# emtiyaz/vmp-for-svae

Hardware: AMD Instinct MI355X
Metric: vmp_step_datapoints_per_sec (higher is better)
Workload: dtype f32

## Files before the change

vmp-for-svae_amd/csrc/vmp_mix.hip:

```cpp
#include "vmp_common.h"
#include "vmp_linalg.h"
#include <stdlib.h>
#include <type_traits>

using namespace vmp;

namespace {

constexpr int TR = 64;
constexpr int LS = 68;
constexpr int MAX_NW = 8;
constexpr int MAX_NW1 = 8;
constexpr int max_nw(int KT) { return KT == 1 ? MAX_NW1 : MAX_NW; }
constexpr int MAX_BLOCKS = 1024;

struct PassArgs {
    const float* x;
    const float* r_in;
    const float* u_in;
    const uint8_t* mask;
    const float* pivot;
    const float* pack;
    float* r_out;
    float* u_out;
    float* logr_out;
    double* partials;
    long long N;
    long long rpw;
    long long rpw_b;
    int K;
    int vec_ok;
    int par_reduce;
#ifdef VMP_DEBUG_TS
    long long* dbg_t;
#endif
};
#ifdef VMP_DEBUG_TS
#define PASS_TS(i) do { if (a.dbg_t && (blockIdx.x == 0 || blockIdx.x == 100) && (threadIdx.x & 63) == 0) { a.dbg_t[(blockIdx.x ? 64 : 0) + (threadIdx.x >> 6) * 8 + (i)] = clock64(); \
    if ((i) == 0 && threadIdx.x == 0) a.dbg_t[(blockIdx.x ? 64 : 0) + 7] = wall_clock64();           \
    if ((i) == 5 && threadIdx.x == 64) a.dbg_t[(blockIdx.x ? 64 : 0) + 8 + 7] = wall_clock64(); } } while (0)
#else
#define PASS_TS(i) do { } while (0)
#endif

#define VMP_DPP2(OP, CTRL)                                                   \
    "v_" OP "_f32_dpp %0, %0, %0 " CTRL " row_mask:0xf bank_mask:0xf\n\t"  \
    "v_" OP "_f32_dpp %1, %1, %1 " CTRL " row_mask:0xf bank_mask:0xf\n\t"  \
    "s_nop 0\n\t"
#define VMP_DPP2_FIRST(OP, CTRL)                                             \
    "v_" OP "_f32_dpp %0, %2, %2 " CTRL " row_mask:0xf bank_mask:0xf\n\t"  \
    "v_" OP "_f32_dpp %1, %3, %3 " CTRL " row_mask:0xf bank_mask:0xf\n\t"  \
    "s_nop 0\n\t"
__device__ __forceinline__ v2f row16_max2(v2f v) {
    float a, b;
    asm("s_nop 1\n\t" VMP_DPP2_FIRST("max", "row_ror:8") VMP_DPP2("max", "row_ror:4") VMP_DPP2("max", "row_ror:2")
// ... 456 lines not shown
#pragma unroll
                for (int kt = 0; kt < KT; ++kt) {
#pragma unroll
                    for (int c = 0; c < 4; ++c) {
                        if constexpr (SMM) dn[kt][c] += (double)nacc[kt][c] + (double)nacs[kt][c];
#pragma unroll
                        for (int ft = 0; ft < FT; ++ft) dacc[kt][ft][c] += (double)acc[kt][ft][c] + (double)acs[kt][ft][c];
                    }
                    nacc[kt] = f32x4{0.f, 0.f, 0.f, 0.f};
                    nacs[kt] = f32x4{0.f, 0.f, 0.f, 0.f};
#pragma unroll
                    for (int ft = 0; ft < FT; ++ft) { acc[kt][ft] = f32x4{0.f, 0.f, 0.f, 0.f}; acs[kt][ft] = f32x4{0.f, 0.f, 0.f, 0.f}; }
                }
            }
        }
        __builtin_amdgcn_wave_barrier();
    }

    PASS_TS(2);
    if constexpr (STATS) pass_epilogue<D, KT, FLAV>(a, smem, dacc, dn, lane, wave, nw);
}


constexpr int AIS = 36;

struct FinArgs {
    const double* partials;
    const double* stats_in;
    int nblk, K, flavour, src, do_post;
    const float *alpha0, *beta0, *m0, *C0, *v0, *kappa;
    const float* pivot;
    float *alpha, *beta, *m, *C, *v, *xbar, *S, *pi, *pack;
    double* pack64;
    double* stats_out;
    double* peer[VMP_EXCH_MAX_RANKS];
    int nranks, rank;
    unsigned long long iter;
    int* status;
#ifdef VMP_DEBUG_TS
    long long* dbg_t;
#endif
};

#ifdef VMP_DEBUG_TS
#define FIN_TS(i) do { if (a.dbg_t && blockIdx.x == 0 && tid == 0) { a.dbg_t[i] = clock64(); if ((i) == 0) a.dbg_t[6] = wall_clock64(); if ((i) == 5) a.dbg_t[7] = wall_clock64(); } } while (0)
#else
#define FIN_TS(i) do { } while (0)
#endif

template <int D>
__device__ void finalize_block(const FinArgs& a, const int k, const int tid, const int nthreads);

template <int D> constexpr int xdl_wave_floats() { return Geo<D>::XROWS * LS + TR * AIS; }

template <int D, int FLAV, bool STATS, int MT = 3>
__device__ __forceinline__ void pass_xdl_body(const PassArgs& a) {
    using G = Geo<D>;
    constexpr int FT = G::FT, KT = 1;
    constexpr bool SMM = (FLAV == VMP_SMM);
    constexpr int DP = (D + 1) / 2;
    extern __shared__ __attribute__((aligned(16))) float smem[];
    const int lane = threadIdx.x & 63, wave = threadIdx.x >> 6, nw = blockDim.x >> 6;
    const int K = a.K;
    PASS_TS(0);
    float* xl = smem + wave * xdl_wave_floats<D>();
    unsigned* ai = reinterpret_cast<unsigned*>(xl + G::XROWS * LS);
    constexpr int ONE = D, ZERO = D + 1;
    const int ppos = (lane & ~15) + 4 * (lane & 3) + ((lane >> 2) & 3);
    xl[ONE * LS + lane] = 1.0f;
    xl[ZERO * LS + lane] = 0.0f;
    {
        u32x4 ones = u32x4{0x3F803F80u, 0x00003F80u, 0u, 0u}, zeros = u32x4{0u, 0u, 0u, 0u};
        *reinterpret_cast<u32x4*>(ai + lane * AIS + 12) = ones;
        *reinterpret_cast<u32x4*>(ai + lane * AIS + 16) = zeros;
    }

    const bool vec = a.vec_ok != 0;
    long long lo, hi;
    if (a.rpw_b == a.rpw) {
        lo = ((long long)blockIdx.x * nw + wave) * a.rpw;
        hi = lo + a.rpw;
    } else {
        const int hw = nw >> 1;
        const long long base = (long long)blockIdx.x * hw * (a.rpw + a.rpw_b);
        lo = wave < hw ? base + wave * a.rpw : base + hw * a.rpw + (wave - hw) * a.rpw_b;
        hi = lo + (wave < hw ? a.rpw : a.rpw_b);
    }
    if (hi > a.N) hi = a.N;
    float xr[D];
    {
        const long long n = lo + lane;
#pragma unroll
        for (int j = 0; j < D; ++j) xr[j] = 0.f;
        if (n < hi) load_row<D>(a.x + n * D, xr, vec);
    }
    const int i16 = lane & 15, kk = lane >> 4;
    float pv[D];
    {
        const float* __restrict__ pp = a.pivot ? a.pivot : a.x;
        const bool hasp = a.pivot != nullptr;
#pragma unroll
        for (int j = 0; j < D; ++j) { const float v = pp[j]; pv[j] = hasp ? v : 0.f; }
    }

    constexpr int NS = D < 4 ? D : 4;
    constexpr int NB = D > 4 ? D - 4 : 0;
    u32x4 Bsm[NS], B1[NB > 0 ? NB : 1], B2[NB > 0 ? NB : 1];
    v2f pch;
    float pua, pub;
    {
        const bool on = i16 < K;
        const float* __restrict__ p = a.pack + (on ? i16 : 0) * G::PACK;
        float raw[G::PACK];
        if (G::PACK % 4 == 0 && (reinterpret_cast<uintptr_t>(a.pack) & 15) == 0) {
#pragma unroll
            for (int j = 0; j < G::PACK / 4; ++j) {
                const float4 q = reinterpret_cast<const float4*>(p)[j];
                raw[4 * j] = q.x; raw[4 * j + 1] = q.y; raw[4 * j + 2] = q.z; raw[4 * j + 3] = q.w;
            }
        } else {
#pragma unroll
            for (int j = 0; j < G::PACK; ++j) raw[j] = p[j];
        }
        pch.x = on ? raw[D + G::TRI] : -INFINITY;
        pch.y = on ? raw[D + G::TRI + 1] : 0.f;
        pua = on ? raw[D + G::TRI + 2] : 0.f;
        pub = on ? raw[D + G::TRI + 3] : 1.f;
#pragma unroll
        for (int i = 0; i < D; ++i) {
            double bi = 0.0;
#pragma unroll
            for (int j = 0; j <= i; ++j) bi -= (double)raw[D + i * (i + 1) / 2 + j] * ((double)raw[j] - (double)pv[j]);
            unsigned tb[3];
            split_bf16<3>(v2f{(float)bi, 0.f}, tb);
            const unsigned bias0 = (tb[0] & 0xffffu) | (tb[1] << 16), bias1 = tb[2] & 0xffffu;
            unsigned th[4] = {0u, 0u, 0u, 0u}, tm[4] = {0u, 0u, 0u, 0u}, tl[4] = {0u, 0u, 0u, 0u};
#pragma unroll
            for (int q = 0; q < DP; ++q) {
                const int j0 = 2 * q, j1 = 2 * q + 1;
                const float wa = j0 <= i ? raw[D + i * (i + 1) / 2 + j0] : 0.f;
                const float wb = (j1 <= i && j1 < D) ? raw[D + i * (i + 1) / 2 + (j1 <= i ? j1 : 0)] : 0.f;
                unsigned t3[3];
                split_bf16<3>(v2f{wa, wb}, t3);
                th[q] = t3[0]; tm[q] = t3[1]; tl[q] = t3[2];
            }
            if (i < NS) {
                const u32x4 w = kk == 0 ? u32x4{th[0], th[1], tm[0], tm[1]}
                              : kk == 1 ? u32x4{th[0], th[1], tl[0], tl[1]}
                              : kk == 2 ? u32x4{th[0], th[1], tm[0], tm[1]}
                                        : u32x4{bias0, bias1, 0u, 0u};
                Bsm[i] = on ? w : u32x4{0u, 0u, 0u, 0u};
            } else {
                const int ib = i - 4;
                const u32x4 w1 = kk == 0 ? u32x4{th[0], th[1], th[2], th[3]} : kk == 1 ? u32x4{bias0, bias1, 0u, 0u}
                               : kk == 2 ? u32x4{tm[0], tm[1], tm[2], tm[3]} : u32x4{th[0], th[1], th[2], th[3]};
                const u32x4 w2 = kk == 0 ? u32x4{tl[0], tl[1], tl[2], tl[3]} : kk == 1 ? u32x4{th[0], th[1], th[2], th[3]}
                               : kk == 2 ? u32x4{tm[0], tm[1], tm[2], tm[3]} : u32x4{0u, 0u, 0u, 0u};
                B1[ib < 0 ? 0 : ib] = on ? w1 : u32x4{0u, 0u, 0u, 0u};
                B2[ib < 0 ? 0 : ib] = on ? w2 : u32x4{0u, 0u, 0u, 0u};
            }
        }
    }
    const int rho = 4 * (i16 & 3) + (i16 >> 2);
    const int offA1 = rho * AIS + (kk == 1 ? 12 : (kk == 3 ? 4 : 0));
    const int offA2 = rho * AIS + (kk == 0 ? 0 : (kk == 1 ? 8 : (kk == 2 ? 4 : 16)));
    const int offA3 = rho * AIS + (kk == 3 ? 12 : 20 + 4 * kk);

    int offA[FT], offB[FT];
#pragma unroll
    for (int ft = 0; ft < FT; ++ft) {
        const int f = ft * 16 + i16;
        int ra = ZERO, rb = ZERO;
        if (f == 0) { ra = ONE; rb = ONE; }
        else if (f <= D) { ra = f - 1; rb = ONE; }
        else if (f < G::F) {
            int p = f - D - 1, d = 0;
            while (p >= D - d) { p -= D - d; ++d; }
            ra = d; rb = d + p;
        }
        offA[ft] = ra * LS + 4 * kk;
        offB[ft] = rb * LS + 4 * kk;
    }

    f32x4 acc[KT][FT], acs[KT][FT];
    double dacc[KT][FT][4];
    double dn[KT][4];
    float nsum = 0.f;
    double dnl = 0.0;
#pragma unroll
    for (int c = 0; c < 4; ++c) dn[0][c] = 0.0;
#pragma unroll
    for (int ft = 0; ft < FT; ++ft) {
        acc[0][ft] = f32x4{0.f, 0.f, 0.f, 0.f};
        acs[0][ft] = f32x4{0.f, 0.f, 0.f, 0.f};
#pragma unroll
// ... 266 lines not shown
        double acc = (i == lane) ? 1.0 : 0.0;
#pragma unroll
        for (int p = 0; p < i; ++p) acc -= readlane_d(row[p], i) * X[p];
        X[i] = acc * rd[i];
    }
}

template <int D>
__device__ void estep_constants(int k, int flavour, double alpha_k, double alpha_sum, double beta_k, double v_k,
                                double logdetP, double kap, double& c, double& h, double& ua, double& ub, double& elp) {
    const double LOG2 = 0.69314718055994530942, PI = 3.14159265358979323846;
    elp = digamma_d(alpha_k) - digamma_d(alpha_sum);
    double sdg = 0.0;
    if (flavour == VMP_GMM) {
        for (int i = 0; i < D; ++i) sdg += digamma_d(0.5 * (v_k + 1.0 + i));
        const double ld = (logdetP > log(1e-20)) ? logdetP : 0.0;
        const double eld = sdg + D * LOG2 + ld;
        c = elp + 0.5 * eld - 0.5 * (D / beta_k);
        h = 0.5; ua = 1.0; ub = 1.0;
    } else {
        for (int i = 0; i < D; ++i) sdg += digamma_d(0.5 * (v_k + i));
        const double eld = sdg + D * LOG2 + logdetP;
        h = 0.5 * (D + kap);
        c = lgamma(0.5 * (D + kap)) - lgamma(0.5 * kap) - 0.5 * D * log(kap * PI) + elp + 0.5 * eld
            - h * (D / beta_k) + log(kap);
        ua = D + kap;
        ub = D / beta_k + kap;
    }
}

constexpr int FIN_THREADS = 1024;
constexpr int FIN_MAX_GROUPS = FIN_THREADS / 64;

__device__ __forceinline__ void st_pack(const FinArgs& a, int idx, double v) {
    a.pack[idx] = (float)v;
    if (a.pack64) a.pack64[idx] = v;
}

template <int D>
__device__ void finalize_block(const FinArgs& a, const int k, const int tid, const int nthreads) {
    using G = Geo<D>;
    __shared__ double part[FIN_MAX_GROUPS][64];
    __shared__ double st[G::SW];
    __shared__ double ntot;
    __shared__ double Ck[D * D], mk[D], sp[D + 4], scal[8];
    __shared__ double alpha0s[VMP_MAX_K];
    const int K = a.K;
    const int FIN_GROUPS = nthreads >> 6;
    const bool post = a.do_post != 0;
    const bool smm = a.flavour == VMP_SMM;
    const double beta0 = post ? (double)a.beta0[k] : 0.0, v0 = post ? (double)a.v0[k] : 0.0;
    const double alpha0 = post ? (double)a.alpha0[k] : 0.0;
    const double kap = (post && smm) ? (double)a.kappa[k] : 0.0;
    bool shifted = (a.src == 0) && (a.pivot != nullptr);
    double m0d = 0.0, m0e = 0.0, C0de = 0.0, cd = 0.0, ce = 0.0;
    if (tid < D * D) {
        const int d = tid / D, e = tid % D;
        if (post) { m0d = a.m0[k * D + d]; m0e = a.m0[k * D + e]; C0de = a.C0[(k * D + d) * D + e]; }
        if (shifted) { cd = a.pivot[d]; ce = a.pivot[e]; }
    }
    if (post && tid < K) alpha0s[tid] = a.alpha0[tid];

    FIN_TS(0);
    if (a.src == 0) {
        constexpr int PX = G::PF + 1;
        const int f = tid & 63, g = tid >> 6;
        const double* __restrict__ mine = a.partials + (long long)k * MAX_BLOCKS * PX;
        for (int lg = g; lg < FIN_MAX_GROUPS; lg += FIN_GROUPS) {
            double s = 0.0;
            for (int b0 = lg; b0 < a.nblk; b0 += FIN_MAX_GROUPS * 16) {
                double v1[16];
                const int fc = f < PX ? f : PX - 1;
#pragma unroll
                for (int i = 0; i < 16; ++i) {
                    const int b = b0 + i * FIN_MAX_GROUPS;
                    const int bc = b < a.nblk ? b : a.nblk - 1;
                    v1[i] = mine[(long long)bc * PX + fc];
                }
#pragma unroll
// ... 122 lines not shown
    const double v_k = smm ? (v0 + Nk) : (v0 + Nk + 1.0);
    FIN_TS(2);
    if (tid < D * D) {
        const int d = tid / D, e = tid % D;
        const double xd = empty ? sx[d] : sx[d] / den, xe = empty ? sx[e] : sx[e] / den;
        const double cen = sxx[d * D + e] - xd * sx[e] - sx[d] * xe + Wk * xd * xe;
        const double Sde = empty ? cen : cen / den;
        const double xrd = empty ? sx[d] + Wk * cd : xd + cd, xre = empty ? sx[e] + Wk * ce : xe + ce;
        const double q0d = xrd - m0d, q0e = xre - m0e;
        const double Cde = C0de + Wk * Sde + (beta0 * Wk / beta_k) * q0d * q0e;
        Ck[d * D + e] = Cde;
        if (a.S) a.S[(k * D + d) * D + e] = (float)Sde;
        if (a.C) a.C[(k * D + d) * D + e] = (float)Cde;
        if (e == 0) {
            const double md = (beta0 * m0d + Wk * xrd) / beta_k;
            mk[d] = md;
            if (a.m) a.m[k * D + d] = (float)md;
            if (a.xbar) a.xbar[k * D + d] = (float)xrd;
        }
    }
    if (tid == 0) {
        if (a.alpha) a.alpha[k] = (float)alpha_k;
        if (a.beta) a.beta[k] = (float)beta_k;
        if (a.v) a.v[k] = (float)v_k;
    }
    __syncthreads();
    FIN_TS(3);
    if (tid < 64) {
        double X[D], sumlog;
        bool ok;
        wave_chol_inverse<D>(Ck, tid, X, sumlog, ok);
        const double sv = ok ? sqrt(v_k) : nan("");
        if (a.pack && tid < D) {
            const int p = k * G::PACK + D;
#pragma unroll
            for (int i = 0; i < D; ++i)
                if (i >= tid) st_pack(a, p + i * (i + 1) / 2 + tid, X[i] * sv);
        }
        if (tid == 0) { scal[0] = -2.0 * sumlog; scal[1] = ok ? 1.0 : 0.0; }
    } else if (tid >= 64 && tid < 64 + D + 2) {
        const int i = tid - 64;
        double arg = 0.5 * (v_k + (smm ? 0.0 : 1.0) + i);
        if (i == D) arg = alpha_k;
        if (i == D + 1) {
            double asum = 0.0;
            for (int j = 0; j < K; ++j) asum += alpha0s[j];
            arg = asum + ntot;
        }
        sp[i] = digamma_d(arg);
    } else if (tid == 128 && smm) {
        sp[D + 2] = lgamma(0.5 * (D + kap)) - lgamma(0.5 * kap);
    }
    __syncthreads();
    FIN_TS(4);
    if (tid == 0) {
        const double LOG2 = 0.69314718055994530942, PI = 3.14159265358979323846;
        const double elp = sp[D] - sp[D + 1];
        double sdg = 0.0;
        for (int i = 0; i < D; ++i) sdg += sp[i];
        double c, h = 0.5, ua = 1.0, ub = 1.0;
        const double logdetP = scal[0];
        if (!smm) {
            const double ld = (logdetP > log(1e-20)) ? logdetP : 0.0;
            c = elp + 0.5 * (sdg + D * LOG2 + ld) - 0.5 * (D / beta_k);
        } else {
            h = 0.5 * (D + kap);
            c = sp[D + 2] - 0.5 * D * log(kap * PI) + elp + 0.5 * (sdg + D * LOG2 + logdetP) - h * (D / beta_k) + log(kap);
            ua = D + kap;
            ub = D / beta_k + kap;
        }
        if (scal[1] == 0.0) c = nan("");
        if (a.pi) a.pi[k] = (float)exp(elp);
        if (a.pack) {
            const int p = k * G::PACK + D + G::TRI;
            const double LOG2E = 1.4426950408889634074;
            st_pack(a, p, c * LOG2E); st_pack(a, p + 1, h * LOG2E); st_pack(a, p + 2, ua); st_pack(a, p + 3, ub);
        }
    }
    if (a.pack && tid < D) st_pack(a, k * G::PACK + tid, mk[tid]);
    FIN_TS(5);
}

template <int D>
__global__ __launch_bounds__(FIN_THREADS) void finalize_kernel(FinArgs a) {
    finalize_block<D>(a, blockIdx.x, threadIdx.x, FIN_THREADS);
}


struct PackArgs {
    int K, flavour;
    const float *alpha, *beta, *m, *P, *v, *kappa;
    float *pack, *pi;
};

template <int D>
__global__ void pack_kernel(PackArgs a) {
    const int k = blockIdx.x * blockDim.x + threadIdx.x;
    if (k >= a.K) return;
    double asum = 0.0;
    for (int j = 0; j < a.K; ++j) asum += a.alpha[j];
    const double v_k = a.v[k];
    double A[D * D], mk[D];
    for (int i = 0; i < D; ++i)
        for (int j = 0; j < D; ++j) {
            const int ri = D - 1 - i, rj = D - 1 - j;
            A[i * D + j] = 0.5 * ((double)a.P[(k * D + ri) * D + rj] + (double)a.P[(k * D + rj) * D + ri]);
        }
    double c = 0, h = 0.5, ua = 1, ub = 1, elp = 0;
    double W[D * D];
    if (chol_lower<D>(A)) {
        double ld = 0.0;
        for (int i = 0; i < D; ++i) ld += log(A[i * D + i]);
// ... 102 lines not shown
int launch_pass_dk(const PassArgs& a, const Plan& p, int flavour, bool estep, bool stats, bool mask, hipStream_t s) {
    dim3 grid(p.blocks), block(p.nw * WAVE);
#define VMP_LAUNCH(FL, E, S, M) \
    hipLaunchKernelGGL((pass_kernel<D, KT, FL, E, S, M>), grid, block, p.lds, s, a)
    if (flavour == VMP_GMM) {
        if (estep && stats) VMP_LAUNCH(VMP_GMM, true, true, false);
        else if (estep && mask) VMP_LAUNCH(VMP_GMM, true, false, true);
        else if (estep) VMP_LAUNCH(VMP_GMM, true, false, false);
        else VMP_LAUNCH(VMP_GMM, false, true, false);
    } else {
        if (estep && stats) VMP_LAUNCH(VMP_SMM, true, true, false);
        else if (estep) VMP_LAUNCH(VMP_SMM, true, false, false);
        else VMP_LAUNCH(VMP_SMM, false, true, false);
    }
#undef VMP_LAUNCH
    return check_launch("pass_kernel");
}

inline bool use_xdl(int K, bool estep, bool mask) { return estep && !mask && K <= 16; }

#ifndef VMP_MOM2_ROWS
#define VMP_MOM2_ROWS (1ll << 16)
#endif
template <int D>
int launch_pass_xdl(const PassArgs& a, const Plan& p, int flavour, bool stats, hipStream_t s) {
    dim3 grid(p.blocks), block(p.nw * WAVE);
#define VMP_LAUNCH_X(FL, S, M) do { \
        if (p.lds > 64 * 1024) { if (const int rc_ = set_dyn_lds(reinterpret_cast<const void*>(pass_xdl_kernel<D, FL, S, M>), p.lds, "pass_xdl_kernel")) return rc_; } \
        hipLaunchKernelGGL((pass_xdl_kernel<D, FL, S, M>), grid, block, p.lds, s, a); } while (0)
    const bool m2 = stats && a.N >= VMP_MOM2_ROWS;
    if (flavour == VMP_GMM) { if (m2) VMP_LAUNCH_X(VMP_GMM, true, 2); else if (stats) VMP_LAUNCH_X(VMP_GMM, true, 3); else VMP_LAUNCH_X(VMP_GMM, false, 3); }
    else { if (m2) VMP_LAUNCH_X(VMP_SMM, true, 2); else if (stats) VMP_LAUNCH_X(VMP_SMM, true, 3); else VMP_LAUNCH_X(VMP_SMM, false, 3); }
#undef VMP_LAUNCH_X
    return check_launch("pass_xdl_kernel");
}

template <int D>
int launch_pass_d(const PassArgs& a, const Plan& p, int flavour, bool estep, bool stats, bool mask, hipStream_t s) {
    if (use_xdl(a.K, estep, mask)) return launch_pass_xdl<D>(a, p, flavour, stats, s);
    const int KT = (a.K + 15) / 16;
    if (KT == 1) return launch_pass_dk<D, 1>(a, p, flavour, estep, stats, mask, s);
    if (KT == 2) return launch_pass_dk<D, 2>(a, p, flavour, estep, stats, mask, s);
    return launch_pass_dk<D, 4>(a, p, flavour, estep, stats, mask, s);
}

#define VMP_DISPATCH_D(D, CALL)            \
    switch (D) {                            \
        case 1: { constexpr int DD = 1; CALL; } break; \
        case 2: { constexpr int DD = 2; CALL; } break; \
        case 3: { constexpr int DD = 3; CALL; } break; \
        case 4: { constexpr int DD = 4; CALL; } break; \
        case 5: { constexpr int DD = 5; CALL; } break; \
        case 6: { constexpr int DD = 6; CALL; } break; \
        case 7: { constexpr int DD = 7; CALL; } break; \
        case 8: { constexpr int DD = 8; CALL; } break; \
        default: break;                     \
    }

int check_dims(int64_t N, int D, int K) {
    if (N <= 0) { set_error("N must be positive (got %lld)", (long long)N); return VMP_E_BADARG; }
    if (D < 1 || D > VMP_MAX_D) { set_error("D=%d outside compiled range 1..%d", D, VMP_MAX_D); return VMP_E_DIM; }
    if (K < 1 || K > VMP_MAX_K) { set_error("K=%d outside compiled range 1..%d", K, VMP_MAX_K); return VMP_E_DIM; }
    return 0;
}

bool aligned16(const void* p) { return (reinterpret_cast<uintptr_t>(p) & 15) == 0; }
// ... 128 lines not shown
            double s = 0.0;
            for (int n = 0; n < nr; ++n) {
                const double rr = (double)ws_[n * K + k];
                const double w = (smm && !isn[q]) ? rr * (double)us_[n * K + k] : rr;
                s = fma(w, (double)xs[n * XS + ia[q]] * (double)xs[n * XS + ib[q]], s);
            }
            acc[q] += s;
        }
    }
    __syncthreads();
    double* nk = reinterpret_cast<double*>(sm);
#pragma unroll
    for (int q = 0; q < ACC_ITEMS; ++q)
        if (ik[q] >= 0 && isn[q]) nk[ik[q]] = acc[q];
    __syncthreads();
    if (threadIdx.x == 0) {
        double t = 0.0;
        for (int k = 0; k < K; ++k) t += nk[k];
        nk[K] = t;
    }
    __syncthreads();
    constexpr int PX = G::PF + 1;
#pragma unroll
    for (int q = 0; q < ACC_ITEMS; ++q) {
        if (ik[q] < 0) continue;
        const int it = (int)threadIdx.x + q * ACC_THREADS, f = it - ik[q] * FP;
        double* row = a.partials + ((long long)ik[q] * MAX_BLOCKS + blockIdx.x) * PX;
        row[f] = acc[q];
        if (f == 0) row[G::PF] = nk[K];
    }
}

constexpr size_t WS_TPACK_WORDS = 16 * (VMP_MAX_D + VMP_MAX_D * (VMP_MAX_D + 1) / 2 + 4);
inline size_t ws_partial_bytes(int D, int K) { return (size_t)MAX_BLOCKS * K * (partial_words(D) + 1) * sizeof(double); }
inline unsigned long long* ws_seq(void* ws, int D, int K) { return reinterpret_cast<unsigned long long*>(static_cast<char*>(ws) + ws_partial_bytes(D, K)); }

}

extern "C" {

#ifdef VMP_DEBUG_TS
void vmp_debug_set_finalize_timestamps(long long* p) { g_dbg_t = p; }
void vmp_debug_set_pass_timestamps(long long* p) { g_dbg_pass = p; }
#endif

int vmp_mix_pack_words(int D) { return pack_words(D); }
int vmp_mix_stats_words(int D) { return stats_words(D); }

size_t vmp_mix_workspace_bytes(int64_t N, int D, int K) {
    (void)N;
    return ws_partial_bytes(D, K) + (WS_TPACK_WORDS + 2) * sizeof(unsigned long long);
}

int vmp_mix_pivot(const float* x, int64_t N, int D, float* pivot_out, void* stream) {
    int rc = check_dims(N, D, 1);
    if (rc) return rc;
    if (!x || !pivot_out) { set_error("vmp_mix_pivot: null pointer"); return VMP_E_BADARG; }
    PivotArgs a{x, N, D, pivot_out};
    hipLaunchKernelGGL(pivot_kernel, dim3(1), dim3(1024), 0, static_cast<hipStream_t>(stream), a);
    return check_launch("pivot_kernel");
}

int vmp_mix_stats(const float* x, const float* r, const float* u, const float* pivot, int64_t N, int D, int K,
                  double* stats, void* ws, size_t ws_bytes, void* stream) {
    int rc = check_dims(N, D, K);
    if (rc) return rc;
    if (!x || !r || !stats || !ws) { set_error("vmp_mix_stats: null pointer"); return VMP_E_BADARG; }
    if (ws_bytes < vmp_mix_workspace_bytes(N, D, K)) { set_error("vmp_mix_stats: workspace too small"); return VMP_E_WS; }
    hipStream_t s = static_cast<hipStream_t>(stream);
    if (N <= SMALL_STATS_MAX_N && !pivot) {
        SmallStatsArgs sa{x, r, u, stats, (int)N, D, K};
        hipLaunchKernelGGL(small_stats_kernel, dim3(K), dim3(SMALL_STATS_GROUPS * 80), 0, s, sa);
        return check_launch("small_stats_kernel");
    }
    const int flavour = u ? VMP_SMM : VMP_GMM;
    PassArgs a{};
    a.x = x; a.r_in = r; a.u_in = u; a.pivot = pivot; a.N = N; a.K = K; a.partials = static_cast<double*>(ws);
    a.vec_ok = aligned16(x) && aligned16(r) && (!u || aligned16(u));
    rc = run_pass(a, D, flavour, false, true, false, s);
    if (rc) return rc;
    FinArgs f{};
    f.partials = a.partials; f.nblk = make_plan(N, D, K, flavour, true).blocks; f.K = K; f.flavour = flavour;
    f.src = 0; f.do_post = 0; f.stats_out = stats; f.pivot = pivot;
    return run_finalize(f, D, s);
}

int vmp_mix_finalize(const double* stats, int D, int K, int flavour, const float* alpha0, const float* beta0,
                     const float* m0, const float* C0, const float* v0, const float* kappa, float* alpha, float* beta,
                     float* m, float* C, float* v, float* xbar, float* S, float* pi, float* pack, void* stream) {
    int rc = check_dims(1, D, K);
    if (rc) return rc;
    if (!stats || !alpha0 || !beta0 || !m0 || !C0 || !v0) { set_error("vmp_mix_finalize: null pointer"); return VMP_E_BADARG; }
    if (flavour == VMP_SMM && !kappa) { set_error("vmp_mix_finalize: SMM needs kappa"); return VMP_E_BADARG; }
    FinArgs f{};
    f.stats_in = stats; f.nblk = 0; f.K = K; f.flavour = flavour; f.src = 1; f.do_post = 1;
    f.alpha0 = alpha0; f.beta0 = beta0; f.m0 = m0; f.C0 = C0; f.v0 = v0; f.kappa = kappa;
    f.alpha = alpha; f.beta = beta; f.m = m; f.C = C; f.v = v; f.xbar = xbar; f.S = S; f.pi = pi; f.pack = pack;
    return run_finalize(f, D, static_cast<hipStream_t>(stream));
}

int vmp_mix_pack_from_params(int D, int K, int flavour, const float* alpha, const float* beta, const float* m,
                             const float* P, const float* v, const float* kappa, float* pack, float* pi, void* stream) {
    int rc = check_dims(1, D, K);
    if (rc) return rc;
    if (!alpha || !beta || !m || !P || !v || !pack) { set_error("vmp_mix_pack_from_params: null pointer"); return VMP_E_BADARG; }
    if (flavour == VMP_SMM && !kappa) { set_error("vmp_mix_pack_from_params: SMM needs kappa"); return VMP_E_BADARG; }
    PackArgs a{K, flavour, alpha, beta, m, P, v, kappa, pack, pi};
    hipStream_t s = static_cast<hipStream_t>(stream);
    rc = -1;
    VMP_DISPATCH_D(D, {
        hipLaunchKernelGGL((pack_kernel<DD>), dim3((K + 63) / 64), dim3(64), 0, s, a);
        rc = check_launch("pack_kernel");
    });
    return rc;
}

int vmp_mix_estep(const float* x, int64_t N, int D, int K, int flavour, const float* pack, const uint8_t* miss_mask,
                  float* r_out, float* u_out, float* logr_out, const float* pivot, double* stats_out, void* ws,
                  size_t ws_bytes, void* stream) {
    int rc = check_dims(N, D, K);
    if (rc) return rc;
    if (!x || !pack || !r_out) { set_error("vmp_mix_estep: null pointer"); return VMP_E_BADARG; }
    if (flavour == VMP_SMM && !u_out) { set_error("vmp_mix_estep: SMM needs u_out"); return VMP_E_BADARG; }
    if (flavour != VMP_GMM && flavour != VMP_SMM) { set_error("vmp_mix_estep: bad flavour %d", flavour); return VMP_E_BADARG; }
    if (miss_mask && (flavour != VMP_GMM || stats_out)) {
        set_error("vmp_mix_estep: miss_mask only with GMM flavour and without fused stats");
        return VMP_E_BADARG;
    }
    if (stats_out && (!ws || ws_bytes < vmp_mix_workspace_bytes(N, D, K))) {
        set_error("vmp_mix_estep: workspace too small for fused stats");
        return VMP_E_WS;
    }
    hipStream_t s = static_cast<hipStream_t>(stream);
    PassArgs a{};
    a.x = x; a.mask = miss_mask; a.pack = pack; a.r_out = r_out; a.u_out = u_out; a.logr_out = logr_out;
    a.pivot = pivot; a.N = N; a.K = K; a.partials = static_cast<double*>(ws);
    a.vec_ok = aligned16(x) && aligned16(r_out) && (!u_out || aligned16(u_out)) && (!logr_out || aligned16(logr_out));
    rc = run_pass(a, D, flavour, true, stats_out != nullptr, miss_mask != nullptr, s);
    if (rc || !stats_out) return rc;
    FinArgs f{};
    f.partials = a.partials; f.nblk = make_plan(N, D, K, flavour, true).blocks; f.K = K; f.flavour = flavour;
    f.src = 0; f.do_post = 0; f.stats_out = stats_out; f.pivot = pivot;
    return run_finalize(f, D, s);
}

int vmp_mix_estep_fused(const float* x, int64_t N, int D, int K, int flavour, const float* pack, float* r_out,
                        float* u_out, float* logr_out, const float* pivot, void* ws, size_t ws_bytes, void* stream) {
    int rc = check_dims(N, D, K);
    if (rc) return rc;
    if (!x || !pack || !r_out || !ws) { set_error("vmp_mix_estep_fused: null pointer"); return VMP_E_BADARG; }
    if (flavour != VMP_GMM && flavour != VMP_SMM) { set_error("vmp_mix_estep_fused: bad flavour %d", flavour); return VMP_E_BADARG; }
    if (flavour == VMP_SMM && !u_out) { set_error("vmp_mix_estep_fused: SMM needs u_out"); return VMP_E_BADARG; }
    if (ws_bytes < vmp_mix_workspace_bytes(N, D, K)) { set_error("vmp_mix_estep_fused: workspace too small"); return VMP_E_WS; }
    PassArgs a{};
    a.x = x; a.pack = pack; a.r_out = r_out; a.u_out = u_out; a.logr_out = logr_out; a.pivot = pivot;
    a.N = N; a.K = K; a.partials = static_cast<double*>(ws);
    a.vec_ok = aligned16(x) && aligned16(r_out) && (!u_out || aligned16(u_out)) && (!logr_out || aligned16(logr_out));
    return run_pass(a, D, flavour, true, true, false, static_cast<hipStream_t>(stream));
}

int vmp_mix_stats_ws(const float* x, const float* r, const float* u, const float* pivot, int64_t N, int D, int K,
                     void* ws, size_t ws_bytes, void* stream) {
    int rc = check_dims(N, D, K);
    if (rc) return rc;
    if (!x || !r || !ws) { set_error("vmp_mix_stats_ws: null pointer"); return VMP_E_BADARG; }
    if (ws_bytes < vmp_mix_workspace_bytes(N, D, K)) { set_error("vmp_mix_stats_ws: workspace too small"); return VMP_E_WS; }
    PassArgs a{};
    a.x = x; a.r_in = r; a.u_in = u; a.pivot = pivot; a.N = N; a.K = K; a.partials = static_cast<double*>(ws);
    a.vec_ok = aligned16(x) && aligned16(r) && (!u || aligned16(u));
    hipError_t e = hipMemsetAsync(ws_seq(ws, D, K), 0, (WS_TPACK_WORDS + 2) * sizeof(unsigned long long), static_cast<hipStream_t>(stream));
    if (e != hipSuccess) { set_error("vmp_mix_stats_ws: hipMemsetAsync: %s", hipGetErrorString(e)); return (int)e; }
    return run_pass(a, D, u ? VMP_SMM : VMP_GMM, false, true, false, static_cast<hipStream_t>(stream));
}

int vmp_mix_stats_ws_accurate(const float* x, const float* r, const float* u, const float* pivot, int64_t N, int D, int K,
                              void* ws, size_t ws_bytes, void* stream) {
    int rc = check_dims(N, D, K);
    if (rc) return rc;
    if (!x || !r || !ws) { set_error("vmp_mix_stats_ws_accurate: null pointer"); return VMP_E_BADARG; }
    if (ws_bytes < vmp_mix_workspace_bytes(N, D, K)) { set_error("vmp_mix_stats_ws_accurate: workspace too small"); return VMP_E_WS; }
    const int blocks = make_plan(N, D, K, u ? VMP_SMM : VMP_GMM, true).blocks;
    AccStatArgs a{x, r, u, pivot, static_cast<double*>(ws), N, (N + blocks - 1) / blocks, K};
    const size_t lds = (size_t)ACC_RS * (D + 1 + 2 * K) * sizeof(float);
    hipStream_t s = static_cast<hipStream_t>(stream);
    hipError_t e = hipMemsetAsync(ws_seq(ws, D, K), 0, (WS_TPACK_WORDS + 2) * sizeof(unsigned long long), s);
    if (e != hipSuccess) { set_error("vmp_mix_stats_ws_accurate: hipMemsetAsync: %s", hipGetErrorString(e)); return (int)e; }
    rc = -1;
    VMP_DISPATCH_D(D, {
        if (lds > 48 * 1024) { if ((rc = set_dyn_lds(reinterpret_cast<const void*>(stats_f64_kernel<DD>), lds, "stats_f64_kernel")) != 0) return rc; }
        hipLaunchKernelGGL((stats_f64_kernel<DD>), dim3(blocks), dim3(ACC_THREADS), lds, s, a);
        rc = check_launch("stats_f64_kernel");
    });
    return rc;
}

int vmp_mix_finalize_exchange(const void* ws, const float* pivot, int64_t N, int D, int K, int flavour, const float* alpha0,
                              const float* beta0, const float* m0, const float* C0, const float* v0, const float* kappa,
                              float* alpha, float* beta, float* m, float* C, float* v, float* xbar, float* S, float* pi,
                              float* pack, double* stats_out, void* const* peers, int nranks, int rank,
                              unsigned long long iteration, int* status, void* stream) {
    int rc = check_dims(N, D, K);
    if (rc) return rc;
    if (!ws || !alpha0 || !beta0 || !m0 || !C0 || !v0 || !peers) { set_error("vmp_mix_finalize_exchange: null pointer"); return VMP_E_BADARG; }
    if (nranks < 1 || nranks > VMP_EXCH_MAX_RANKS || rank < 0 || rank >= nranks) { set_error("vmp_mix_finalize_exchange: bad rank / nranks"); return VMP_E_BADARG; }
    if (flavour == VMP_SMM && !kappa) { set_error("vmp_mix_finalize_exchange: SMM needs kappa"); return VMP_E_BADARG; }
    FinArgs f{};
    f.partials = static_cast<const double*>(ws);
    f.nblk = make_plan(N, D, K, flavour, true).blocks;
    f.K = K; f.flavour = flavour; f.src = 0;
    f.do_post = (alpha || beta || m || C || v || xbar || S || pi || pack) ? 1 : 0;
    f.alpha0 = alpha0; f.beta0 = beta0; f.m0 = m0; f.C0 = C0; f.v0 = v0; f.kappa = kappa;
    f.alpha = alpha; f.beta = beta; f.m = m; f.C = C; f.v = v; f.xbar = xbar; f.S = S; f.pi = pi; f.pack = pack;
    f.stats_out = stats_out; f.pivot = pivot;
    for (int g = 0; g < nranks; ++g) {
        if (!peers[g]) { set_error("vmp_mix_finalize_exchange: peers[%d] is null", g); return VMP_E_BADARG; }
        f.peer[g] = static_cast<double*>(peers[g]);
    }
    f.nranks = nranks; f.rank = rank; f.iter = iteration; f.status = status;
    return run_finalize(f, D, static_cast<hipStream_t>(stream));
}

int vmp_mix_finalize_ws(const void* ws, const float* pivot, int64_t N, int D, int K, int flavour, const float* alpha0, const float* beta0,
                        const float* m0, const float* C0, const float* v0, const float* kappa, float* alpha,
                        float* beta, float* m, float* C, float* v, float* xbar, float* S, float* pi, float* pack,
                        double* stats_out, void* stream) {
    int rc = check_dims(N, D, K);
    if (rc) return rc;
    if (!ws || !alpha0 || !beta0 || !m0 || !C0 || !v0) { set_error("vmp_mix_finalize_ws: null pointer"); return VMP_E_BADARG; }
    if (flavour == VMP_SMM && !kappa) { set_error("vmp_mix_finalize_ws: SMM needs kappa"); return VMP_E_BADARG; }
    FinArgs f{};
    f.partials = static_cast<const double*>(ws);
    f.nblk = make_plan(N, D, K, flavour, true).blocks;
    f.K = K; f.flavour = flavour; f.src = 0;
    f.do_post = (alpha || beta || m || C || v || xbar || S || pi || pack) ? 1 : 0;
    f.alpha0 = alpha0; f.beta0 = beta0; f.m0 = m0; f.C0 = C0; f.v0 = v0; f.kappa = kappa;
    f.alpha = alpha; f.beta = beta; f.m = m; f.C = C; f.v = v; f.xbar = xbar; f.S = S; f.pi = pi; f.pack = pack;
    f.stats_out = stats_out; f.pivot = pivot;
    return run_finalize(f, D, static_cast<hipStream_t>(stream));
}

int vmp_mix_finalize_ws64(const void* ws, const float* pivot, int64_t N, int D, int K, int flavour, const float* alpha0, const float* beta0,
                          const float* m0, const float* C0, const float* v0, const float* kappa, float* alpha,
                          float* beta, float* m, float* C, float* v, float* xbar, float* S, float* pi, float* pack, double* pack64,
                          double* stats_out, void* stream) {
    int rc = check_dims(N, D, K);
    if (rc) return rc;
    if (!ws || !alpha0 || !beta0 || !m0 || !C0 || !v0 || !pack || !pack64) { set_error("vmp_mix_finalize_ws64: null pointer"); return VMP_E_BADARG; }
    if (flavour == VMP_SMM && !kappa) { set_error("vmp_mix_finalize_ws64: SMM needs kappa"); return VMP_E_BADARG; }
    FinArgs f{};
    f.partials = static_cast<const double*>(ws);
    f.nblk = make_plan(N, D, K, flavour, true).blocks;
    f.K = K; f.flavour = flavour; f.src = 0; f.do_post = 1;
    f.alpha0 = alpha0; f.beta0 = beta0; f.m0 = m0; f.C0 = C0; f.v0 = v0; f.kappa = kappa;
    f.alpha = alpha; f.beta = beta; f.m = m; f.C = C; f.v = v; f.xbar = xbar; f.S = S; f.pi = pi; f.pack = pack; f.pack64 = pack64;
    f.stats_out = stats_out; f.pivot = pivot;
    return run_finalize(f, D, static_cast<hipStream_t>(stream));
}

int vmp_mix_estep_accurate(const float* x, int64_t N, int D, int K, int flavour, const double* pack64, float* r_out, float* u_out,
                           float* logr_out, void* stream) {
    int rc = check_dims(N, D, K);
    if (rc) return rc;
    if (!x || !pack64 || !r_out) { set_error("vmp_mix_estep_accurate: null pointer"); return VMP_E_BADARG; }
    if (flavour != VMP_GMM && flavour != VMP_SMM) { set_error("vmp_mix_estep_accurate: bad flavour %d", flavour); return VMP_E_BADARG; }
    if (flavour == VMP_SMM && !u_out) { set_error("vmp_mix_estep_accurate: SMM needs u_out"); return VMP_E_BADARG; }
    AccArgs a{x, pack64, r_out, u_out, logr_out, N, K};
    long long blocks = (N + 255) / 256;
    if (blocks > 2048) blocks = 2048;
    const size_t lds = (size_t)K * pack_words(D) * sizeof(double);
    hipStream_t s = static_cast<hipStream_t>(stream);
    VMP_DISPATCH_D(D, {
        if (flavour == VMP_SMM) hipLaunchKernelGGL((estep_f64_kernel<DD, true>), dim3((int)blocks), dim3(256), lds, s, a);
        else hipLaunchKernelGGL((estep_f64_kernel<DD, false>), dim3((int)blocks), dim3(256), lds, s, a);
    });
    return check_launch("estep_f64_kernel");
}

int vmp_mix_iterate(const float* x, int64_t N, int D, int K, int flavour, const float* alpha0, const float* beta0,
                    const float* m0, const float* C0, const float* v0, const float* kappa, const float* pivot,
                    float* r, float* u, float* alpha, float* beta, float* m, float* C, float* v, float* xbar, float* S,
                    float* pi, float* pack, void* ws, size_t ws_bytes, int iterations, void* stream) {
    if (iterations < 0 || !pack) { set_error("vmp_mix_iterate: bad argument"); return VMP_E_BADARG; }
    for (int it = 0; it < iterations; ++it) {
        int rc = vmp_mix_finalize_ws(ws, pivot, N, D, K, flavour, alpha0, beta0, m0, C0, v0, kappa, alpha, beta, m, C, v,
                                     xbar, S, pi, pack, nullptr, stream);
        if (rc) return rc;
        rc = vmp_mix_estep_fused(x, N, D, K, flavour, pack, r, u, nullptr, pivot, ws, ws_bytes, stream);
        if (rc) return rc;
// ... 6 lines not shown
```

Baseline: 20.83 billion.

## Precompute E-step MFMA operand image in finalize and reuse it in fused pass

The finalize kernel now builds the per-lane bf16-split MFMA operands (Bsm/B1/B2 and scalar params) once per component and writes them, plus a checksum row of the pack and pivot, into an extra workspace region. The fused E-step pass loads this image and checks it against the live pack and pivot. If every lane matches, it skips rebuilding the operands (the triangular bias computation in double and the bf16 splits). This removes per-block prologue arithmetic at the cost of extra workspace, loads and a validation compare, and it only applies when K<=16 and the workspace is large enough.

```diff
diff --git a/vmp-for-svae_amd/csrc/vmp_mix.hip b/vmp-for-svae_amd/csrc/vmp_mix.hip
--- a/vmp-for-svae_amd/csrc/vmp_mix.hip
+++ b/vmp-for-svae_amd/csrc/vmp_mix.hip
@@ -21,6 +21,7 @@
     const uint8_t* mask;
     const float* pivot;
     const float* pack;
+    const unsigned* image;
     float* r_out;
     float* u_out;
     float* logr_out;
@@ -543,6 +544,8 @@
     const float* pivot;
     float *alpha, *beta, *m, *C, *v, *xbar, *S, *pi, *pack;
     double* pack64;
+    unsigned* image;
+    const unsigned long long* image_tag;
     double* stats_out;
     double* peer[VMP_EXCH_MAX_RANKS];
     int nranks, rank;
@@ -563,6 +566,76 @@
 __device__ void finalize_block(const FinArgs& a, const int k, const int tid, const int nthreads);
 
 template <int D> constexpr int xdl_wave_floats() { return Geo<D>::XROWS * LS + TR * AIS; }
+
+template <int D> struct EOps {
+    static constexpr int NS = D < 4 ? D : 4;
+    static constexpr int NB = D > 4 ? D - 4 : 0;
+    u32x4 Bsm[NS], B1[NB > 0 ? NB : 1], B2[NB > 0 ? NB : 1];
+    v2f pch;
+    float pua, pub;
+};
+template <int D>
+__device__ __forceinline__ void build_estep_operands(const float (&raw)[Geo<D>::PACK], const float (&pv)[D], const bool on, const int kk, EOps<D>& o) {
+    using G = Geo<D>;
+    constexpr int NS = EOps<D>::NS, DP = (D + 1) / 2;
+    o.pch.x = on ? raw[D + G::TRI] : -INFINITY;
+    o.pch.y = on ? raw[D + G::TRI + 1] : 0.f;
+    o.pua = on ? raw[D + G::TRI + 2] : 0.f;
+    o.pub = on ? raw[D + G::TRI + 3] : 1.f;
+#pragma unroll
+    for (int i = 0; i < D; ++i) {
+        double bi = 0.0;
+#pragma unroll
+        for (int j = 0; j <= i; ++j) bi -= (double)raw[D + i * (i + 1) / 2 + j] * ((double)raw[j] - (double)pv[j]);
+        unsigned tb[3];
+        split_bf16<3>(v2f{(float)bi, 0.f}, tb);
+        const unsigned bias0 = (tb[0] & 0xffffu) | (tb[1] << 16), bias1 = tb[2] & 0xffffu;
+        unsigned th[4] = {0u, 0u, 0u, 0u}, tm[4] = {0u, 0u, 0u, 0u}, tl[4] = {0u, 0u, 0u, 0u};
+#pragma unroll
+        for (int q = 0; q < DP; ++q) {
+            const int j0 = 2 * q, j1 = 2 * q + 1;
+            const float wa = j0 <= i ? raw[D + i * (i + 1) / 2 + j0] : 0.f;
+            const float wb = (j1 <= i && j1 < D) ? raw[D + i * (i + 1) / 2 + (j1 <= i ? j1 : 0)] : 0.f;
+            unsigned t3[3];
+            split_bf16<3>(v2f{wa, wb}, t3);
+            th[q] = t3[0]; tm[q] = t3[1]; tl[q] = t3[2];
+        }
+        if (i < NS) {
+            const u32x4 w = kk == 0 ? u32x4{th[0], th[1], tm[0], tm[1]}
+                          : kk == 1 ? u32x4{th[0], th[1], tl[0], tl[1]}
+                          : kk == 2 ? u32x4{th[0], th[1], tm[0], tm[1]}
+                                    : u32x4{bias0, bias1, 0u, 0u};
+            o.Bsm[i < NS ? i : 0] = on ? w : u32x4{0u, 0u, 0u, 0u};
+        } else {
+            const int ib = i - 4;
+            const u32x4 w1 = kk == 0 ? u32x4{th[0], th[1], th[2], th[3]} : kk == 1 ? u32x4{bias0, bias1, 0u, 0u}
+                           : kk == 2 ? u32x4{tm[0], tm[1], tm[2], tm[3]} : u32x4{th[0], th[1], th[2], th[3]};
+            const u32x4 w2 = kk == 0 ? u32x4{tl[0], tl[1], tl[2], tl[3]} : kk == 1 ? u32x4{th[0], th[1], th[2], th[3]}
+                           : kk == 2 ? u32x4{tm[0], tm[1], tm[2], tm[3]} : u32x4{0u, 0u, 0u, 0u};
+            o.B1[ib < 0 ? 0 : ib] = on ? w1 : u32x4{0u, 0u, 0u, 0u};
+            o.B2[ib < 0 ? 0 : ib] = on ? w2 : u32x4{0u, 0u, 0u, 0u};
+        }
+    }
+}
+
+constexpr unsigned IMG_MAGIC = 0x45494d47u;
+template <int D> struct EImg {
+    static constexpr int NOP = EOps<D>::NS + 2 * EOps<D>::NB;
+    static constexpr int SLOT = 4 * (NOP + 1);
+    static constexpr int CW = (Geo<D>::PACK + D + 2 + 3) & ~3;
+    static constexpr int CHK = 64 * SLOT;
+    static constexpr int WORDS = CHK + 16 * CW;
+};
+template <int D>
+__device__ __forceinline__ void store_estep_image(unsigned* image, const int lane, const EOps<D>& o) {
+    constexpr int NS = EOps<D>::NS, NB = EOps<D>::NB;
+    u32x4* slot = reinterpret_cast<u32x4*>(image + lane * EImg<D>::SLOT);
+#pragma unroll
+    for (int i = 0; i < NS; ++i) slot[i] = o.Bsm[i];
+#pragma unroll
+    for (int i = 0; i < NB; ++i) { slot[NS + i] = o.B1[i]; slot[NS + NB + i] = o.B2[i]; }
+    slot[NS + 2 * NB] = u32x4{__float_as_uint(o.pch.x), __float_as_uint(o.pch.y), __float_as_uint(o.pua), __float_as_uint(o.pub)};
+}
 
 template <int D, int FLAV, bool STATS, int MT = 3>
 __device__ __forceinline__ void pass_xdl_body(const PassArgs& a) {
@@ -614,11 +687,8 @@
         for (int j = 0; j < D; ++j) { const float v = pp[j]; pv[j] = hasp ? v : 0.f; }
     }
 
-    constexpr int NS = D < 4 ? D : 4;
-    constexpr int NB = D > 4 ? D - 4 : 0;
-    u32x4 Bsm[NS], B1[NB > 0 ? NB : 1], B2[NB > 0 ? NB : 1];
-    v2f pch;
-    float pua, pub;
+    constexpr int NS = EOps<D>::NS, NB = EOps<D>::NB;
+    EOps<D> eo;
     {
         const bool on = i16 < K;
         const float* __restrict__ p = a.pack + (on ? i16 : 0) * G::PACK;
@@ -633,45 +703,45 @@
 #pragma unroll
             for (int j = 0; j < G::PACK; ++j) raw[j] = p[j];
         }
-        pch.x = on ? raw[D + G::TRI] : -INFINITY;
-        pch.y = on ? raw[D + G::TRI + 1] : 0.f;
-        pua = on ? raw[D + G::TRI + 2] : 0.f;
-        pub = on ? raw[D + G::TRI + 3] : 1.f;
-#pragma unroll
-        for (int i = 0; i < D; ++i) {
-            double bi = 0.0;
-#pragma unroll
-            for (int j = 0; j <= i; ++j) bi -= (double)raw[D + i * (i + 1) / 2 + j] * ((double)raw[j] - (double)pv[j]);
-            unsigned tb[3];
-            split_bf16<3>(v2f{(float)bi, 0.f}, tb);
-            const unsigned bias0 = (tb[0] & 0xffffu) | (tb[1] << 16), bias1 = tb[2] & 0xffffu;
-            unsigned th[4] = {0u, 0u, 0u, 0u}, tm[4] = {0u, 0u, 0u, 0u}, tl[4] = {0u, 0u, 0u, 0u};
-#pragma unroll
-            for (int q = 0; q < DP; ++q) {
-                const int j0 = 2 * q, j1 = 2 * q + 1;
-                const float wa = j0 <= i ? raw[D + i * (i + 1) / 2 + j0] : 0.f;
-                const float wb = (j1 <= i && j1 < D) ? raw[D + i * (i + 1) / 2 + (j1 <= i ? j1 : 0)] : 0.f;
-                unsigned t3[3];
-                split_bf16<3>(v2f{wa, wb}, t3);
-                th[q] = t3[0]; tm[q] = t3[1]; tl[q] = t3[2];
-            }
-            if (i < NS) {
-                const u32x4 w = kk == 0 ? u32x4{th[0], th[1], tm[0], tm[1]}
-                              : kk == 1 ? u32x4{th[0], th[1], tl[0], tl[1]}
-                              : kk == 2 ? u32x4{th[0], th[1], tm[0], tm[1]}
-                                        : u32x4{bias0, bias1, 0u, 0u};
-                Bsm[i] = on ? w : u32x4{0u, 0u, 0u, 0u};
-            } else {
-                const int ib = i - 4;
-                const u32x4 w1 = kk == 0 ? u32x4{th[0], th[1], th[2], th[3]} : kk == 1 ? u32x4{bias0, bias1, 0u, 0u}
-                               : kk == 2 ? u32x4{tm[0], tm[1], tm[2], tm[3]} : u32x4{th[0], th[1], th[2], th[3]};
-                const u32x4 w2 = kk == 0 ? u32x4{tl[0], tl[1], tl[2], tl[3]} : kk == 1 ? u32x4{th[0], th[1], th[2], th[3]}
-                               : kk == 2 ? u32x4{tm[0], tm[1], tm[2], tm[3]} : u32x4{0u, 0u, 0u, 0u};
-                B1[ib < 0 ? 0 : ib] = on ? w1 : u32x4{0u, 0u, 0u, 0u};
-                B2[ib < 0 ? 0 : ib] = on ? w2 : u32x4{0u, 0u, 0u, 0u};
-            }
-        }
-    }
+        bool have = false;
+        if constexpr (STATS) {
+            if (a.image) {
+                using I = EImg<D>;
+                const u32x4* __restrict__ slot = reinterpret_cast<const u32x4*>(a.image + lane * I::SLOT);
+                const u32x4* __restrict__ chk = reinterpret_cast<const u32x4*>(a.image + I::CHK + i16 * I::CW);
+                u32x4 ops[I::NOP + 1], cw[I::CW / 4];
+#pragma unroll
+                for (int j = 0; j < I::NOP + 1; ++j) ops[j] = slot[j];
+#pragma unroll
+                for (int j = 0; j < I::CW / 4; ++j) cw[j] = chk[j];
+                unsigned diff = 0u;
+#pragma unroll
+                for (int j = 0; j < G::PACK; ++j) diff |= cw[j >> 2][j & 3] ^ __float_as_uint(raw[j]);
+#pragma unroll
+                for (int j = 0; j < D; ++j) diff |= cw[(G::PACK + j) >> 2][(G::PACK + j) & 3] ^ __float_as_uint(pv[j]);
+                if (!on) diff = 0u;
+                diff |= cw[(G::PACK + D) >> 2][(G::PACK + D) & 3] ^ (IMG_MAGIC ^ (unsigned)D);
+                diff |= cw[(G::PACK + D + 1) >> 2][(G::PACK + D + 1) & 3] ^ (unsigned)K;
+                have = __all(diff == 0u) != 0;
+                if (have) {
+#pragma unroll
+                    for (int i = 0; i < NS; ++i) eo.Bsm[i] = ops[i];
+#pragma unroll
+                    for (int i = 0; i < NB; ++i) { eo.B1[i] = ops[NS + i]; eo.B2[i] = ops[NS + NB + i]; }
+                    const u32x4 sc = ops[NS + 2 * NB];
+                    eo.pch = v2f{__uint_as_float(sc[0]), __uint_as_float(sc[1])};
+                    eo.pua = __uint_as_float(sc[2]);
+                    eo.pub = __uint_as_float(sc[3]);
+                }
+            }
+        }
+        if (!have) build_estep_operands<D>(raw, pv, on, kk, eo);
+    }
+    const u32x4 (&Bsm)[NS] = eo.Bsm;
+    const u32x4 (&B1)[NB > 0 ? NB : 1] = eo.B1;
+    const u32x4 (&B2)[NB > 0 ? NB : 1] = eo.B2;
+    const v2f pch = eo.pch;
+    const float pua = eo.pua, pub = eo.pub;
     const int rho = 4 * (i16 & 3) + (i16 >> 2);
     const int offA1 = rho * AIS + (kk == 1 ? 12 : (kk == 3 ? 4 : 0));
     const int offA2 = rho * AIS + (kk == 0 ? 0 : (kk == 1 ? 8 : (kk == 2 ? 4 : 16)));
@@ -1004,8 +1074,12 @@
 constexpr int FIN_THREADS = 1024;
 constexpr int FIN_MAX_GROUPS = FIN_THREADS / 64;
 
-__device__ __forceinline__ void st_pack(const FinArgs& a, int idx, double v) {
+constexpr unsigned long long WS_IMAGE_TAG = 0xA5A5A5A5A5A5A5A5ull;
+
+__device__ __forceinline__ void st_pack(const FinArgs& a, float* row, int base, int j, double v) {
+    const int idx = base + j;
     a.pack[idx] = (float)v;
+    row[j] = (float)v;
     if (a.pack64) a.pack64[idx] = v;
 }
 
@@ -1017,6 +1091,7 @@
     __shared__ double ntot;
     __shared__ double Ck[D * D], mk[D], sp[D + 4], scal[8];
     __shared__ double alpha0s[VMP_MAX_K];
+    __shared__ float prow[G::PACK];
     const int K = a.K;
     const int FIN_GROUPS = nthreads >> 6;
     const bool post = a.do_post != 0;
@@ -1205,10 +1280,9 @@
         wave_chol_inverse<D>(Ck, tid, X, sumlog, ok);
         const double sv = ok ? sqrt(v_k) : nan("");
         if (a.pack && tid < D) {
-            const int p = k * G::PACK + D;
 #pragma unroll
             for (int i = 0; i < D; ++i)
-                if (i >= tid) st_pack(a, p + i * (i + 1) / 2 + tid, X[i] * sv);
+                if (i >= tid) st_pack(a, prow, k * G::PACK, D + i * (i + 1) / 2 + tid, X[i] * sv);
         }
         if (tid == 0) { scal[0] = -2.0 * sumlog; scal[1] = ok ? 1.0 : 0.0; }
     } else if (tid >= 64 && tid < 64 + D + 2) {
@@ -1245,12 +1319,41 @@
         if (scal[1] == 0.0) c = nan("");
         if (a.pi) a.pi[k] = (float)exp(elp);
         if (a.pack) {
-            const int p = k * G::PACK + D + G::TRI;
+            const int p = D + G::TRI;
             const double LOG2E = 1.4426950408889634074;
-            st_pack(a, p, c * LOG2E); st_pack(a, p + 1, h * LOG2E); st_pack(a, p + 2, ua); st_pack(a, p + 3, ub);
-        }
-    }
-    if (a.pack && tid < D) st_pack(a, k * G::PACK + tid, mk[tid]);
+            st_pack(a, prow, k * G::PACK, p, c * LOG2E); st_pack(a, prow, k * G::PACK, p + 1, h * LOG2E);
+            st_pack(a, prow, k * G::PACK, p + 2, ua); st_pack(a, prow, k * G::PACK, p + 3, ub);
+        }
+    }
+    if (a.pack && tid < D) st_pack(a, prow, k * G::PACK, tid, mk[tid]);
+    if (a.pack && a.image && *a.image_tag == WS_IMAGE_TAG && k < 16 && K <= 16) {
+        using I = EImg<D>;
+        __syncthreads();
+        float pvf[D];
+#pragma unroll
+        for (int j = 0; j < D; ++j) pvf[j] = a.pivot ? a.pivot[j] : 0.f;
+        const bool mine = tid < 4, off = k == 0 && tid >= 64 && tid < 128 && ((tid & 15) >= K);
+        if (mine || off) {
+            float raw[G::PACK];
+#pragma unroll
+            for (int j = 0; j < G::PACK; ++j) raw[j] = prow[j];
+            EOps<D> eo;
+            build_estep_operands<D>(raw, pvf, mine, mine ? tid : (tid - 64) >> 4, eo);
+            store_estep_image<D>(a.image, mine ? tid * 16 + k : tid - 64, eo);
+        }
+        for (int kr = k; kr < 16; kr += (k == 0 ? 1 : 16)) {
+            if (kr != k && kr < K) continue;
+            unsigned* row = a.image + I::CHK + kr * I::CW;
+            for (int j = tid; j < I::CW; j += nthreads) {
+                unsigned w = 0u;
+                if (j < G::PACK) w = __float_as_uint(prow[j]);
+                else if (j < G::PACK + D) w = __float_as_uint(a.pivot ? a.pivot[j - G::PACK] : 0.f);
+                else if (j == G::PACK + D) w = IMG_MAGIC ^ (unsigned)D;
+                else if (j == G::PACK + D + 1) w = (unsigned)K;
+                row[j] = w;
+            }
+        }
+    }
     FIN_TS(5);
 }
 
@@ -1419,6 +1522,7 @@
     if (flavour == VMP_GMM) { if (m2) VMP_LAUNCH_X(VMP_GMM, true, 2); else if (stats) VMP_LAUNCH_X(VMP_GMM, true, 3); else VMP_LAUNCH_X(VMP_GMM, false, 3); }
     else { if (m2) VMP_LAUNCH_X(VMP_SMM, true, 2); else if (stats) VMP_LAUNCH_X(VMP_SMM, true, 3); else VMP_LAUNCH_X(VMP_SMM, false, 3); }
 #undef VMP_LAUNCH_X
+#undef VMP_LAUNCH_X
     return check_launch("pass_xdl_kernel");
 }
 
@@ -1613,8 +1717,23 @@
 }
 
 constexpr size_t WS_TPACK_WORDS = 16 * (VMP_MAX_D + VMP_MAX_D * (VMP_MAX_D + 1) / 2 + 4);
+constexpr size_t WS_IMAGE_BYTES = (size_t)EImg<VMP_MAX_D>::WORDS * sizeof(unsigned);
 inline size_t ws_partial_bytes(int D, int K) { return (size_t)MAX_BLOCKS * K * (partial_words(D) + 1) * sizeof(double); }
+inline size_t ws_min_bytes(int D, int K) { return ws_partial_bytes(D, K) + (WS_TPACK_WORDS + 2) * sizeof(unsigned long long); }
+inline size_t ws_full_bytes(int D, int K) { return ws_min_bytes(D, K) + WS_IMAGE_BYTES; }
 inline unsigned long long* ws_seq(void* ws, int D, int K) { return reinterpret_cast<unsigned long long*>(static_cast<char*>(ws) + ws_partial_bytes(D, K)); }
+inline unsigned* ws_image(void* ws, int D, int K) { return reinterpret_cast<unsigned*>(static_cast<char*>(ws) + ws_min_bytes(D, K)); }
+int seed_ws(void* ws, size_t ws_bytes, int D, int K, hipStream_t s, const char* who) {
+    hipError_t e = hipMemsetAsync(ws_seq(ws, D, K), 0, (WS_TPACK_WORDS + 2) * sizeof(unsigned long long), s);
+    if (e == hipSuccess && ws_bytes >= ws_full_bytes(D, K)) e = hipMemsetAsync(ws_seq(ws, D, K), (int)(WS_IMAGE_TAG & 0xff), sizeof(unsigned long long), s);
+    if (e != hipSuccess) { set_error("%s: hipMemsetAsync: %s", who, hipGetErrorString(e)); return (int)e; }
+    return 0;
+}
+inline void fin_image(FinArgs& f, const void* ws, int D, int K) {
+    void* w = const_cast<void*>(ws);
+    f.image = (f.pack && K <= 16) ? ws_image(w, D, K) : nullptr;
+    f.image_tag = ws_seq(w, D, K);
+}
 
 }
 
@@ -1630,7 +1749,7 @@
 
 size_t vmp_mix_workspace_bytes(int64_t N, int D, int K) {
     (void)N;
-    return ws_partial_bytes(D, K) + (WS_TPACK_WORDS + 2) * sizeof(unsigned long long);
+    return ws_full_bytes(D, K);
 }
 
 int vmp_mix_pivot(const float* x, int64_t N, int D, float* pivot_out, void* stream) {
@@ -1647,7 +1766,7 @@
     int rc = check_dims(N, D, K);
     if (rc) return rc;
     if (!x || !r || !stats || !ws) { set_error("vmp_mix_stats: null pointer"); return VMP_E_BADARG; }
-    if (ws_bytes < vmp_mix_workspace_bytes(N, D, K)) { set_error("vmp_mix_stats: workspace too small"); return VMP_E_WS; }
+    if (ws_bytes < ws_min_bytes(D, K)) { set_error("vmp_mix_stats: workspace too small"); return VMP_E_WS; }
     hipStream_t s = static_cast<hipStream_t>(stream);
     if (N <= SMALL_STATS_MAX_N && !pivot) {
         SmallStatsArgs sa{x, r, u, stats, (int)N, D, K};
@@ -1708,7 +1827,7 @@
         set_error("vmp_mix_estep: miss_mask only with GMM flavour and without fused stats");
         return VMP_E_BADARG;
     }
-    if (stats_out && (!ws || ws_bytes < vmp_mix_workspace_bytes(N, D, K))) {
+    if (stats_out && (!ws || ws_bytes < ws_min_bytes(D, K))) {
         set_error("vmp_mix_estep: workspace too small for fused stats");
         return VMP_E_WS;
     }
@@ -1732,10 +1851,11 @@
     if (!x || !pack || !r_out || !ws) { set_error("vmp_mix_estep_fused: null pointer"); return VMP_E_BADARG; }
     if (flavour != VMP_GMM && flavour != VMP_SMM) { set_error("vmp_mix_estep_fused: bad flavour %d", flavour); return VMP_E_BADARG; }
     if (flavour == VMP_SMM && !u_out) { set_error("vmp_mix_estep_fused: SMM needs u_out"); return VMP_E_BADARG; }
-    if (ws_bytes < vmp_mix_workspace_bytes(N, D, K)) { set_error("vmp_mix_estep_fused: workspace too small"); return VMP_E_WS; }
+    if (ws_bytes < ws_min_bytes(D, K)) { set_error("vmp_mix_estep_fused: workspace too small"); return VMP_E_WS; }
     PassArgs a{};
     a.x = x; a.pack = pack; a.r_out = r_out; a.u_out = u_out; a.logr_out = logr_out; a.pivot = pivot;
     a.N = N; a.K = K; a.partials = static_cast<double*>(ws);
+    if (K <= 16 && ws_bytes >= ws_full_bytes(D, K) && aligned16(ws)) a.image = ws_image(ws, D, K);
     a.vec_ok = aligned16(x) && aligned16(r_out) && (!u_out || aligned16(u_out)) && (!logr_out || aligned16(logr_out));
     return run_pass(a, D, flavour, true, true, false, static_cast<hipStream_t>(stream));
 }
@@ -1745,12 +1865,12 @@
     int rc = check_dims(N, D, K);
     if (rc) return rc;
     if (!x || !r || !ws) { set_error("vmp_mix_stats_ws: null pointer"); return VMP_E_BADARG; }
-    if (ws_bytes < vmp_mix_workspace_bytes(N, D, K)) { set_error("vmp_mix_stats_ws: workspace too small"); return VMP_E_WS; }
+    if (ws_bytes < ws_min_bytes(D, K)) { set_error("vmp_mix_stats_ws: workspace too small"); return VMP_E_WS; }
     PassArgs a{};
     a.x = x; a.r_in = r; a.u_in = u; a.pivot = pivot; a.N = N; a.K = K; a.partials = static_cast<double*>(ws);
     a.vec_ok = aligned16(x) && aligned16(r) && (!u || aligned16(u));
-    hipError_t e = hipMemsetAsync(ws_seq(ws, D, K), 0, (WS_TPACK_WORDS + 2) * sizeof(unsigned long long), static_cast<hipStream_t>(stream));
-    if (e != hipSuccess) { set_error("vmp_mix_stats_ws: hipMemsetAsync: %s", hipGetErrorString(e)); return (int)e; }
+    rc = seed_ws(ws, ws_bytes, D, K, static_cast<hipStream_t>(stream), "vmp_mix_stats_ws");
+    if (rc) return rc;
     return run_pass(a, D, u ? VMP_SMM : VMP_GMM, false, true, false, static_cast<hipStream_t>(stream));
 }
 
@@ -1759,13 +1879,13 @@
     int rc = check_dims(N, D, K);
     if (rc) return rc;
     if (!x || !r || !ws) { set_error("vmp_mix_stats_ws_accurate: null pointer"); return VMP_E_BADARG; }
-    if (ws_bytes < vmp_mix_workspace_bytes(N, D, K)) { set_error("vmp_mix_stats_ws_accurate: workspace too small"); return VMP_E_WS; }
+    if (ws_bytes < ws_min_bytes(D, K)) { set_error("vmp_mix_stats_ws_accurate: workspace too small"); return VMP_E_WS; }
     const int blocks = make_plan(N, D, K, u ? VMP_SMM : VMP_GMM, true).blocks;
     AccStatArgs a{x, r, u, pivot, static_cast<double*>(ws), N, (N + blocks - 1) / blocks, K};
     const size_t lds = (size_t)ACC_RS * (D + 1 + 2 * K) * sizeof(float);
     hipStream_t s = static_cast<hipStream_t>(stream);
-    hipError_t e = hipMemsetAsync(ws_seq(ws, D, K), 0, (WS_TPACK_WORDS + 2) * sizeof(unsigned long long), s);
-    if (e != hipSuccess) { set_error("vmp_mix_stats_ws_accurate: hipMemsetAsync: %s", hipGetErrorString(e)); return (int)e; }
+    rc = seed_ws(ws, ws_bytes, D, K, s, "vmp_mix_stats_ws_accurate");
+    if (rc) return rc;
     rc = -1;
     VMP_DISPATCH_D(D, {
         if (lds > 48 * 1024) { if ((rc = set_dyn_lds(reinterpret_cast<const void*>(stats_f64_kernel<DD>), lds, "stats_f64_kernel")) != 0) return rc; }
@@ -1798,6 +1918,7 @@
         f.peer[g] = static_cast<double*>(peers[g]);
     }
     f.nranks = nranks; f.rank = rank; f.iter = iteration; f.status = status;
+    fin_image(f, ws, D, K);
     return run_finalize(f, D, static_cast<hipStream_t>(stream));
 }
 
@@ -1817,6 +1938,7 @@
     f.alpha0 = alpha0; f.beta0 = beta0; f.m0 = m0; f.C0 = C0; f.v0 = v0; f.kappa = kappa;
     f.alpha = alpha; f.beta = beta; f.m = m; f.C = C; f.v = v; f.xbar = xbar; f.S = S; f.pi = pi; f.pack = pack;
     f.stats_out = stats_out; f.pivot = pivot;
+    fin_image(f, ws, D, K);
     return run_finalize(f, D, static_cast<hipStream_t>(stream));
 }
 
@@ -1835,6 +1957,7 @@
     f.alpha0 = alpha0; f.beta0 = beta0; f.m0 = m0; f.C0 = C0; f.v0 = v0; f.kappa = kappa;
     f.alpha = alpha; f.beta = beta; f.m = m; f.C = C; f.v = v; f.xbar = xbar; f.S = S; f.pi = pi; f.pack = pack; f.pack64 = pack64;
     f.stats_out = stats_out; f.pivot = pivot;
+    fin_image(f, ws, D, K);
     return run_finalize(f, D, static_cast<hipStream_t>(stream));
 }
 
```

New measurement: 18.80 billion. 9.7% lower.
